# FrancescoScotti/Quadruped_gait_generation_ISMPC

Hardware: AMD Instinct MI355X
Metric: ISMPC QP solves/s (batch, N=100 horizon) (higher is better)
Workload: dtype f64; 1 GPU; Formulation B (MPCSolver::solve), trot plan Controller.cpp:89-97, N=100, S=35, F=10, fp64, global batch 65536 (65536 instances/GPU), nominal pre-roll + perturbation (SURVEY 8d); horizon=100, global_batch=65536, batch_per_gpu=65536

## Files before the change

quadruped_gait_generation_ismpc_amd/csrc/ismpc_b_common.hpp:

```cpp
#pragma once
#include <hip/hip_runtime.h>
#include <cmath>
#include "ismpc_tables.hpp"
#include "ismpc_wave_prims.hpp"

namespace {

using namespace ismpc_wave;

struct DevConst {
    int N, NP, NPs, S, F, nmid, npat, Fmax, rows, tick_divisor;
    double dt, cdt, mass, g, h_des, half_run, half_first, q_p, q_u, q_v, z_lo, z_hi, gate, eta;
    double inv_mass, dt_over_mass, inv_eta, sim_div, cdt_over_dt;
    const double *Hinv, *W, *midx, *midy, *midz, *tailx, *taily, *ftsp_t;
    const int *e_lo, *ne;
    const double *vtab, *tz, *tg, *dU, *SdU, *Wt, *SW;
    int flat;
    const double *HSt, *SHSt;
    const DevConst* sets; int nsets;
    const int* order;
    int* zflag;
    int* zseen;
    double* zpool; int* zbusy;
    int zslots, zcap, zldsq; size_t zstride;
    const double *vq;
    const double *tzg;
    const double *midxy;
    const double *vqT;
    const double *tzgT;
};

struct M2 { double a, b, c, d; };
__device__ __forceinline__ M2 mul(const M2& x, const M2& y)
{
    M2 r;
    r.a = fma(x.a, y.a, x.b * y.c); r.b = fma(x.a, y.b, x.b * y.d);
    r.c = fma(x.c, y.a, x.d * y.c); r.d = fma(x.c, y.b, x.d * y.d);
    return r;
}
template <int LANE>
__device__ __forceinline__ M2 readlane_m2(const M2& y)
{
    return (M2){readlane64<LANE>(y.a), readlane64<LANE>(y.b), readlane64<LANE>(y.c), readlane64<LANE>(y.d)};
}

__device__ __forceinline__ void sinhc_coshc(double w, double& P, double& Q)
{
    if (__builtin_expect(w <= 0.25, 1)) {
        P = 1.0 / 1307674368000.0;
        P = fma(P, w, 1.0 / 6227020800.0);
        P = fma(P, w, 1.0 / 39916800.0);
        P = fma(P, w, 1.0 / 362880.0);
        P = fma(P, w, 1.0 / 5040.0);
        P = fma(P, w, 1.0 / 120.0);
        P = fma(P, w, 1.0 / 6.0);
        P = fma(P, w, 1.0);
        Q = 1.0 / 20922789888000.0;
        Q = fma(Q, w, 1.0 / 87178291200.0);
        Q = fma(Q, w, 1.0 / 479001600.0);
        Q = fma(Q, w, 1.0 / 3628800.0);
        Q = fma(Q, w, 1.0 / 40320.0);
        Q = fma(Q, w, 1.0 / 720.0);
        Q = fma(Q, w, 1.0 / 24.0);
        Q = fma(Q, w, 0.5);
    } else {
        const double x = sqrt(w);
        P = sinh(x) / x;
        Q = (cosh(x) - 1.0) / w;
    }
}

__host__ __device__ inline size_t zscratch_bytes(int batch) { return 4 * (size_t)batch + 16; }
__device__ __forceinline__ int* zlist_of(unsigned char* zmark, int) { return reinterpret_cast<int*>(zmark); }
struct Walk { double sim; int mpc, ctl, fc; };
__device__ __forceinline__ Walk load_walk(const DevConst& c, const ismpc_tick_in* rec, int rollout_frame)
{
    Walk w; w.sim = rec->simulation_time; w.mpc = rec->mpc_iter; w.ctl = rec->control_iter; w.fc = rec->footstep_counter;
    if (rollout_frame >= 0) {
        if (w.fc >= 0 && w.fc < c.rows && w.sim >= c.ftsp_t[w.fc] - 1) { w.ctl = 0; w.mpc = 0; w.fc = w.fc + 1; }
        w.sim = (double)rollout_frame;
    }
    return w;
}
__device__ __forceinline__ int gate_tick(const DevConst& c, const Walk& w, int& idx)
{
    idx = 0;
    if ((w.ctl % c.tick_divisor) != 0) return ISMPC_ST_TICK_SKIPPED;
    const double t = (c.sim_div == 1.0) ? w.sim : w.sim / c.sim_div;
    if (!(t > -1.0) || !(t < 2.0e9)) return ISMPC_ST_BAD_INDEX;
    idx = (int)t;
    if (idx < 0 || idx + 2 * c.N > c.nmid || w.mpc < 0) return ISMPC_ST_BAD_INDEX;
// ... 49 lines not shown
```

quadruped_gait_generation_ismpc_amd/csrc/ismpc_b_group.hpp:

```cpp
#pragma once
#include "ismpc_b_affine.hpp"

namespace {

template <int CTRL, int BANK_MASK>
__device__ __forceinline__ double dpp64b(double old, double src)
{
    const int lo = __builtin_amdgcn_update_dpp(__double2loint(old), __double2loint(src), CTRL, 0xf, BANK_MASK, false);
    const int hi = __builtin_amdgcn_update_dpp(__double2hiint(old), __double2hiint(src), CTRL, 0xf, BANK_MASK, false);
    return __hiloint2double(hi, lo);
}
template <int CTRL, bool BOUND_ZERO>
__device__ __forceinline__ double dpp64n(double src)
{
    const int lo = __builtin_amdgcn_mov_dpp(__double2loint(src), CTRL, 0xf, 0xf, BOUND_ZERO);
    const int hi = __builtin_amdgcn_mov_dpp(__double2hiint(src), CTRL, 0xf, 0xf, BOUND_ZERO);
    return __hiloint2double(hi, lo);
}
template <int LPI> struct Grp;
template <> struct Grp<16> {
    static constexpr int STEPS = 4;
    __device__ static __forceinline__ double sum(double v)
    {
        v += dpp64n<0x121, false>(v); v += dpp64n<0x122, false>(v); v += dpp64n<0x124, false>(v); v += dpp64n<0x128, false>(v);
// ... 59 lines not shown
    }
    template <int K> __device__ static __forceinline__ double shl0(double v, int li)
    {
        if constexpr (K == 2) return dpp64b<0x104, 0x5>(0.0, v);
        else { const double t = dpp64n<0x100 + (1 << K), true>(v); return (li + (1 << K) < 8) ? t : 0.0; }
    }
    __device__ static __forceinline__ double bcast0(double v)
    {
        v = dpp64b<0x000, 0xf>(v, v); v = dpp64b<0x114, 0xa>(v, v);
        return v;
    }
    __device__ static __forceinline__ double next_or(double fill, double v, int li)
    {
        const double t = dppv<0x101, 0xf, false>(fill, v);
        return (li == 7) ? fill : t;
    }
};
template <int LPI, int K>
__device__ __forceinline__ void grp_scan_step(M2& y, int li)
{
    if constexpr (LPI == 32 && K == 4) {
        const bool g1 = (threadIdx.x & 32) != 0, low = li < 16;
        const double ya = g1 ? readlane64<48>(y.a) : readlane64<16>(y.a), yb = g1 ? readlane64<48>(y.b) : readlane64<16>(y.b);
        const double yc = g1 ? readlane64<48>(y.c) : readlane64<16>(y.c), yd = g1 ? readlane64<48>(y.d) : readlane64<16>(y.d);
        const double ta = low ? ya - 1.0 : 0.0, tb = low ? yb : 0.0, tc = low ? yc : 0.0, td = low ? yd - 1.0 : 0.0;
        M2 r;
        r.a = fma(ta, y.a, fma(tb, y.c, y.a)); r.b = fma(ta, y.b, fma(tb, y.d, y.b));
        r.c = fma(tc, y.a, fma(td, y.c, y.c)); r.d = fma(tc, y.b, fma(td, y.d, y.d));
        y = r;
    } else
    if constexpr (K < Grp<LPI>::STEPS) {
        const double ta = Grp<LPI>::template shl0<K>(y.a - 1.0, li), tb = Grp<LPI>::template shl0<K>(y.b, li);
        const double tc = Grp<LPI>::template shl0<K>(y.c, li), td = Grp<LPI>::template shl0<K>(y.d - 1.0, li);
        M2 r;
        r.a = fma(ta, y.a, fma(tb, y.c, y.a)); r.b = fma(ta, y.b, fma(tb, y.d, y.b));
        r.c = fma(tc, y.a, fma(td, y.c, y.c)); r.d = fma(tc, y.b, fma(td, y.d, y.d));
        y = r;
    }
}

template <int R> constexpr int midm() { return R | 1; }
template <int R, int LPI> constexpr int wave_lds_double2() { return (64 / LPI) * LPI * midm<R>(); }
template <int R, int LPI> constexpr int wave_lds_double2_fb() { return wave_lds_double2<R, LPI>() > (Z_LDS_DOUBLES + 1) / 2 ? wave_lds_double2<R, LPI>() : (Z_LDS_DOUBLES + 1) / 2; }

#ifndef ISMPC_KF_INLINE
#define ISMPC_KF_INLINE 0
#endif
#ifndef ISMPC_KF_MAIN
#define ISMPC_KF_MAIN 0
#endif
#ifndef ISMPC_KF_ROLLOUT
#define ISMPC_KF_ROLLOUT 0
#endif
template <int R, int LPI, int KF, bool SW = false>
__device__ __forceinline__ bool tick_group_core(const DevConst& c, const int lane, const QState& s, QOut& o, double* __restrict__ u_traj_inst,
                                                double2* __restrict__ lds_wave)
{
    constexpr int NT = ismpc::Tables::NT;
    const int N = c.N;
    const int li = lane & (LPI - 1);
    const double dt = c.dt;
    const Walk& w = s.w;
    const double x0 = s.x, y0 = s.y, z0 = s.z, xd0 = s.xd, yd0 = s.yd, zd0 = s.zd;
    const DevConst* P = SW ? c.sets + (s.ps >= 0 ? s.ps : 0) : nullptr;
    const double* p_vqT = SW ? P->vqT : c.vqT;
    const double p_z_lo = SW ? P->z_lo : c.z_lo, p_z_hi = SW ? P->z_hi : c.z_hi;
    const double p_inv_mass = SW ? P->inv_mass : c.inv_mass, p_inv_eta = SW ? P->inv_eta : c.inv_eta;
    const double p_half_run = SW ? P->half_run : c.half_run, p_half_first = SW ? P->half_first : c.half_first;
    const double* p_tailx = SW ? P->tailx : c.tailx; const double* p_taily = SW ? P->taily : c.taily;
    const double p_dt_over_mass = SW ? P->dt_over_mass : c.dt_over_mass, p_h_des = SW ? P->h_des : c.h_des;
    int idx;
    const int gate_status = gate_tick(c, w, idx) | ((SW && s.ps < 0) ? ISMPC_ST_BAD_INDEX : 0);
    int status = gate_status;
    const bool run = gate_status == 0;
    if (!run) idx = 0;
    const int n0 = li * R;
    STAMP_DECL;
    STAMP(1);

    const int pat = (run && w.fc > 1 && w.mpc < c.npat) ? w.mpc : c.npat;
    const double2* T = reinterpret_cast<const double2*>(p_vqT) + (size_t)pat * (R * 3 * LPI) + li;
    constexpr int MIDM = midm<R>();
    double2* Lm = lds_wave + (lane / LPI) * (LPI * MIDM);
#pragma unroll
    for (int k = 0; k < R; ++k) {
        const int j = k * LPI + li;
        Lm[(j / R) * MIDM + (j % R)] = reinterpret_cast<const double2*>(c.midxy)[min(idx + j, c.nmid - 1)];
    }
    double u[R], su[R];
    double smin = INFINITY, smax = -INFINITY;
#pragma unroll
    for (int r = 0; r < R; ++r) {
        const double2 t01 = T[(3 * r) * LPI], t23 = T[(3 * r + 1) * LPI], t45 = T[(3 * r + 2) * LPI];
        u[r] = fma(zd0, t23.x, fma(z0, t01.y, t01.x));
        su[r] = fma(zd0, t45.y, fma(z0, t45.x, t23.y));
        if (n0 + r < N) { smin = fmin(smin, su[r]); smax = fmax(smax, su[r]); }
    }
    if (!c.flat) {
        int elo = 0, ne = 0;
        if (pat < c.npat) { elo = c.e_lo[pat]; ne = c.ne[pat]; }
        const int pp = pat < c.npat ? pat : 0;
        int nemax = 0;
#pragma unroll
        for (int g = 0; g < 64; g += LPI) nemax = max(nemax, __builtin_amdgcn_readlane(ne, g));
        const double* dUr = (SW ? P->dU : c.dU) + (size_t)idx * NT;
        const double* sUr = (SW ? P->SdU : c.SdU) + (size_t)idx * NT;
        double du[R], ds[R];
#pragma unroll
        for (int r = 0; r < R; ++r) { du[r] = dUr[n0 + r]; ds[r] = sUr[n0 + r]; }
        for (int e = 0; e < nemax; ++e) {
            const bool on = e < ne;
            const double ue = on ? dUr[elo + e] : 0.0;
            const double* wr = (SW ? P->Wt : c.Wt) + ((size_t)pp * c.Fmax + (on ? e : 0)) * NT + n0;
            const double* sr = (SW ? P->SW : c.SW) + ((size_t)pp * c.Fmax + (on ? e : 0)) * NT + n0;
#pragma unroll
            for (int r = 0; r < R; ++r) { du[r] = fma(-wr[r], ue, du[r]); ds[r] = fma(-sr[r], ue, ds[r]); }
        }
        smin = INFINITY; smax = -INFINITY;
#pragma unroll
        for (int r = 0; r < R; ++r) {
            const int n = n0 + r;
            u[r] += du[r]; su[r] += ds[r];
            if (n >= elo && n < elo + ne) u[r] = 0.0;
            if (n < N) { smin = fmin(smin, su[r]); smax = fmax(smax, su[r]); }
        }
    }
    const double zlo_t = p_z_lo - 1e-11 * fmax(1.0, fabs(p_z_lo)), zhi_t = p_z_hi + 1e-11 * fmax(1.0, fabs(p_z_hi));
    const bool viol = smin < zlo_t || smax > zhi_t;
    const unsigned long long vmask = __builtin_amdgcn_ballot_w64(viol);
    const bool deferred = run && (((vmask >> (lane & (64 - LPI))) & ((1ull << LPI) - 1ull)) != 0ull);
    if (deferred) status |= ISMPC_ST_Z_INEQ_ACTIVE;

    double ch1[R], s1[R], s2[R], lam0_l = 0.0;
    bool big = false, mid = false;
    {
        double wv_[R], le_[R];
#pragma unroll
        for (int r = 0; r < R; ++r) {
            const double2 tq = reinterpret_cast<const double2*>(c.tzgT)[r * LPI + li];
            const double zpos = su[r] + fma(tq.x, zd0, z0) + tq.y;
            const double zacc = fma(p_inv_mass, u[r], -c.g);
            const double lam = (c.g + zacc) * frcp(zpos);
            if (r == 0) lam0_l = lam;
            le_[r] = (lam < c.gate) ? 0.0 : lam;
            const double dtn = (n0 + r < N) ? dt : 0.0;
            wv_[r] = le_[r] * dtn * dtn;
            s1[r] = dtn;
            big = big || (wv_[r] > 0.25);
            mid = mid || (wv_[r] > 0.004);
        }
        if (__builtin_amdgcn_ballot_w64(mid) == 0) {
#pragma unroll
            for (int r = 0; r < R; ++r) {
                const double wv = wv_[r];
                double P = 1.0 / 5040.0, Q = 1.0 / 40320.0;
                P = fma(P, wv, 1.0 / 120.0);         Q = fma(Q, wv, 1.0 / 720.0);
                P = fma(P, wv, 1.0 / 6.0);           Q = fma(Q, wv, 1.0 / 24.0);
                P = fma(P, wv, 1.0);                 Q = fma(Q, wv, 0.5);
                ch1[r] = wv * Q; s1[r] = s1[r] * P; s2[r] = le_[r] * s1[r];
            }
        } else {
            const bool gmid = ((__builtin_amdgcn_ballot_w64(mid) >> (lane & (64 - LPI))) & ((LPI == 64) ? ~0ull : ((1ull << LPI) - 1ull))) != 0ull;
#pragma unroll
            for (int r = 0; r < R; ++r) {
                const double wv = wv_[r], dtn = s1[r];
                double P = 1.0 / 1307674368000.0, Q = 1.0 / 20922789888000.0;
                P = fma(P, wv, 1.0 / 6227020800.0);  Q = fma(Q, wv, 1.0 / 87178291200.0);
                P = fma(P, wv, 1.0 / 39916800.0);    Q = fma(Q, wv, 1.0 / 479001600.0);
                P = fma(P, wv, 1.0 / 362880.0);      Q = fma(Q, wv, 1.0 / 3628800.0);
                P = gmid ? fma(P, wv, 1.0 / 5040.0) : 1.0 / 5040.0;   Q = gmid ? fma(Q, wv, 1.0 / 40320.0) : 1.0 / 40320.0;
                P = fma(P, wv, 1.0 / 120.0);         Q = fma(Q, wv, 1.0 / 720.0);
                P = fma(P, wv, 1.0 / 6.0);           Q = fma(Q, wv, 1.0 / 24.0);
                P = fma(P, wv, 1.0);                 Q = fma(Q, wv, 0.5);
                ch1[r] = wv * Q; s1[r] = dtn * P; s2[r] = le_[r] * s1[r];
                if (__builtin_amdgcn_ballot_w64(big) != 0 && wv > 0.25) {
                    const double x = sqrt(wv);
                    ch1[r] = cosh(x) - 1.0; s1[r] = dtn * (sinh(x) / x); s2[r] = le_[r] * s1[r];
                }
            }
        }
    }
    M2 Y = (M2){1.0 + ch1[0], s1[0], s2[0], 1.0 + ch1[0]};
#pragma unroll
    for (int r = 1; r < R; ++r) Y = mul((M2){1.0 + ch1[r], s1[r], s2[r], 1.0 + ch1[r]}, Y);
    STAMP(2);
    grp_scan_step<LPI, 0>(Y, li); grp_scan_step<LPI, 1>(Y, li); grp_scan_step<LPI, 2>(Y, li); grp_scan_step<LPI, 3>(Y, li);
    grp_scan_step<LPI, 4>(Y, li);
    const double ie = p_inv_eta;
    const double cva = fma(ie, Y.c, Y.a), cvb = fma(ie, Y.d, Y.b);
    double c0 = Grp<LPI>::next_or(1.0, cva, li), c1 = Grp<LPI>::next_or(ie, cvb, li);
    double a[R];
#pragma unroll
    for (int r = R - 1; r >= 0; --r) {
        a[r] = -fma(c0, ch1[r], c1 * s2[r]);
        const double k0 = fma(c0, ch1[r], fma(c1, s2[r], c0)), k1 = fma(c1, ch1[r], fma(c0, s1[r], c1));
        c0 = k0; c1 = k1;
    }
    const double h = (w.fc > 1) ? p_half_run : p_half_first;
    double q0 = 0.0, s_ax = 0.0, s_ay = 0.0, mx0 = 0.0, my0 = 0.0;
    __builtin_amdgcn_fence(__ATOMIC_SEQ_CST, "wavefront"); __builtin_amdgcn_wave_barrier();
#pragma unroll
    for (int r = 0; r < R; ++r) {
        const int n = n0 + r;
        const double2 mq = Lm[li * MIDM + r];
        const double mx = (n < N) ? mq.x : 0.0, my = (n < N) ? mq.y : 0.0;
        if (r == 0) { mx0 = mx; my0 = my; }
        q0 = fma(a[r], a[r], q0); s_ax = fma(a[r], mx, s_ax); s_ay = fma(a[r], my, s_ay);
    }
    q0 = Grp<LPI>::sum(q0); s_ax = Grp<LPI>::sum(s_ax); s_ay = Grp<LPI>::sum(s_ay);
    const double bpx = Grp<LPI>::bcast0((p_tailx[idx] - fma(cva, x0, cvb * xd0)) - s_ax);
    const double bpy = Grp<LPI>::bcast0((p_taily[idx] - fma(cva, y0, cvb * yd0)) - s_ay);
    const double sgx = (bpx < 0.0) ? -1.0 : 1.0, sgy = (bpy < 0.0) ? -1.0 : 1.0;
    STAMP(3);
    const double Tq[2] = { fabs(bpx), fabs(bpy) };
    const double iq0 = frcp(q0);
    double tau[2] = { Tq[0] * iq0, Tq[1] * iq0 };
    int its[2] = {1, 1}, prev[2] = {0, 0};
    bool live[2] = {true, true};
    int st3 = 0;
    if (!(q0 > 0.0)) {
#pragma unroll
        for (int ax = 0; ax < 2; ++ax) {
            tau[ax] = (Tq[ax] > 0.0) ? INFINITY : 0.0;
            if (Tq[ax] > 1e-300) st3 |= (ax == 0 ? ISMPC_ST_X_INFEASIBLE : ISMPC_ST_Y_INFEASIBLE);
        }
    }
    if constexpr (KF == 0) {
        for (int it = 0; it < N + 2; ++it) {
            if (__builtin_amdgcn_ballot_w64(live[0] || live[1]) == 0ull) break;
#pragma unroll
            for (int ax = 0; ax < 2; ++ax) {
                if (__builtin_amdgcn_ballot_w64(live[ax]) == 0ull) continue;
                int cl = 0;
#pragma unroll
                for (int r = 0; r < R; ++r) cl += (tau[ax] * fabs(a[r]) >= h) ? 1 : 0;
                const int cnt = Grp<LPI>::sum_i(cl);
                if (live[ax] && cnt == prev[ax]) live[ax] = false;
                if (__builtin_amdgcn_ballot_w64(live[ax]) == 0ull) continue;
                double ssat = 0.0, qfree = 0.0;
#pragma unroll
                for (int r = 0; r < R; ++r) {
                    const double ab = fabs(a[r]);
                    const bool sat = tau[ax] * ab >= h;
                    const double ms = sat ? 1.0 : 0.0, mf = sat ? 0.0 : 1.0;
                    ssat = fma(ms, ab, ssat); qfree = fma(mf, a[r] * a[r], qfree);
                }
                ssat = Grp<LPI>::sum(ssat); qfree = Grp<LPI>::sum(qfree);
                if (live[ax]) {
                    ++its[ax];
                    const double rem = fma(-h, ssat, Tq[ax]);
                    if (!(qfree > 0.0)) {
                        if (rem > fma(h * ssat, 1e-12, 1e-300)) st3 |= (ax == 0 ? ISMPC_ST_X_INFEASIBLE : ISMPC_ST_Y_INFEASIBLE);
                        tau[ax] = INFINITY; live[ax] = false;
                    } else {
                        const double tn = rem * frcp(qfree);
                        if (!(tn > tau[ax])) live[ax] = false;
                        else { tau[ax] = tn; prev[ax] = cnt; }
                    }
                }
            }
        }
    } else {
        for (int it = 0; it < N + 2; ++it) {
            if (__builtin_amdgcn_ballot_w64(live[0] || live[1]) == 0ull) break;
            int cl[2] = {0, 0};
            double ssat[2] = {0.0, 0.0}, qfree[2] = {0.0, 0.0};
#pragma unroll
            for (int ax = 0; ax < 2; ++ax) {
#pragma unroll
                for (int r = 0; r < R; ++r) {
                    const bool sat = tau[ax] * fabs(a[r]) >= h;
                    cl[ax] += sat ? 1 : 0; ssat[ax] += sat ? fabs(a[r]) : 0.0;
                    const double a2 = a[r] * a[r]; qfree[ax] += sat ? 0.0 : a2;
                }
            }
            const int cnt0 = Grp<LPI>::sum_i(cl[0]), cnt1 = Grp<LPI>::sum_i(cl[1]);
            ssat[0] = Grp<LPI>::sum(ssat[0]); ssat[1] = Grp<LPI>::sum(ssat[1]);
            qfree[0] = Grp<LPI>::sum(qfree[0]); qfree[1] = Grp<LPI>::sum(qfree[1]);
#pragma unroll
            for (int ax = 0; ax < 2; ++ax) {
                const int cnt = ax == 0 ? cnt0 : cnt1;
                if (live[ax] && cnt == prev[ax]) live[ax] = false;
                if (live[ax]) {
                    ++its[ax];
                    const double rem = fma(-h, ssat[ax], Tq[ax]);
                    if (!(qfree[ax] > 0.0)) {
                        if (rem > fma(h * ssat[ax], 1e-12, 1e-300)) st3 |= (ax == 0 ? ISMPC_ST_X_INFEASIBLE : ISMPC_ST_Y_INFEASIBLE);
                        tau[ax] = INFINITY; live[ax] = false;
                    } else {
                        const double tn = rem * frcp(qfree[ax]);
                        if (!(tn > tau[ax])) live[ax] = false;
                        else { tau[ax] = tn; prev[ax] = cnt; }
                    }
                }
            }
        }
    }

    STAMP(4);
    o.x = x0; o.y = y0; o.z = z0; o.xd = xd0; o.yd = yd0; o.zd = zd0;
    o.uz0 = 0.0; o.ux0 = 0.0; o.uy0 = 0.0; o.itx = 0; o.ity = 0;
    if (li == 0 && run) {
        o.uz0 = u[0];
        o.z = fma(dt, zd0, z0);
        o.zd = fma(p_dt_over_mass, o.uz0, zd0) - dt * c.g;
        if (isnan(o.z)) { o.z = p_h_des; status |= ISMPC_ST_Z_NAN; }
        if (isnan(o.zd)) { o.zd = 0.0; status |= ISMPC_ST_Z_NAN; }
        const double A0a = 1.0 + ch1[0], A0b = s1[0], A0c = s2[0];
        if (lam0_l > c.gate) {
            status |= st3; o.itx = its[0]; o.ity = its[1];
            const double sa0 = (a[0] < 0.0) ? -1.0 : 1.0;
            o.ux0 = fma(sgx * sa0, (fabs(a[0]) > 0.0) ? fmin(tau[0] * fabs(a[0]), h) : 0.0, mx0);
            o.uy0 = fma(sgy * sa0, (fabs(a[0]) > 0.0) ? fmin(tau[1] * fabs(a[0]), h) : 0.0, my0);
        } else status |= ISMPC_ST_FLIGHT;
        o.x  = fma(1.0 - A0a, o.ux0, fma(A0a, x0, A0b * xd0));
        o.xd = fma(-A0c, o.ux0, fma(A0c, x0, A0a * xd0));
        o.y  = fma(1.0 - A0a, o.uy0, fma(A0a, y0, A0b * yd0));
        o.yd = fma(-A0c, o.uy0, fma(A0c, y0, A0a * yd0));
    }
    o.status = status;
    if (u_traj_inst) {
        const bool stage3 = run && Grp<LPI>::bcast0(lam0_l) > c.gate;
#pragma unroll
        for (int r = 0; r < R; ++r) {
            const int n = n0 + r;
            if (n < N) {
                double vx = 0.0, vy = 0.0;
                if (stage3) {
                    const double sa = (a[r] < 0.0) ? -1.0 : 1.0;
                    vx = fma(sgx * sa, (fabs(a[r]) > 0.0) ? fmin(tau[0] * fabs(a[r]), h) : 0.0, c.midx[idx + n]);
                    vy = fma(sgy * sa, (fabs(a[r]) > 0.0) ? fmin(tau[1] * fabs(a[r]), h) : 0.0, c.midy[idx + n]);
                }
                u_traj_inst[n] = run ? u[r] : 0.0; u_traj_inst[N + n] = vx; u_traj_inst[2 * N + n] = vy;
            }
        }
    }
    return deferred;
}

template <int R, int LPI, int KF, bool SW = false>
__device__ __forceinline__ bool tick_group_body(const DevConst& c, const int gi_raw, const int batch, const int lane,
                                                const ismpc_tick_in* __restrict__ in_ro, ismpc_tick_in* state_rw,
                                                ismpc_tick_out* __restrict__ out, double* __restrict__ u_traj,
                                                int rollout_frame, unsigned char* zmark, int launch_id, double2* __restrict__ lds_wave, int* zlist = nullptr)
{
    const bool valid = gi_raw < batch;
    const int gi = valid ? gi_raw : batch - 1;
    STAMP_DECL;
    STAMP(0);
    const ismpc_tick_in* rec = ((rollout_frame >= 0) ? state_rw : in_ro) + gi;
    QState s;
    s.w = load_walk(c, rec, rollout_frame);
    s.x = rec->com_pos[0]; s.y = rec->com_pos[1]; s.z = rec->com_pos[2];
    s.xd = rec->com_vel[0]; s.yd = rec->com_vel[1]; s.zd = rec->com_vel[2];
    s.ps = 0;
    if (SW) { const int ps = rec->reserved; s.ps = (ps >= 0 && ps < c.nsets) ? ps : -1; }
    QOut o;
    const bool deferred = tick_group_core<R, LPI, KF, SW>(c, lane, s, o, (u_traj && valid) ? u_traj + (size_t)gi * 3 * c.N : nullptr, lds_wave);
    if ((lane & (LPI - 1)) == 0 && valid) {
        if (out) store_record(out + gi, o);
        if (deferred) {
            if (c.zseen) *c.zseen = launch_id;
            if (zlist) { const int slot = atomicAdd(c.zflag, 1); if (slot < batch) zlist[slot] = gi; }
        }
        if (rollout_frame >= 0 && !deferred) store_feedback(c, state_rw + gi, o, s.w);
    }
    STAMP(5);
    return deferred && valid;
}

#ifndef ISMPC_QUAD_WAVES
#define ISMPC_QUAD_WAVES 4
#endif
__device__ __forceinline__ int sweep_vblock(int b, int nb)
{
    const int q = nb >> 3, r = nb & 7, x = b & 7;
    return x * q + min(x, r) + (b >> 3);
}
template <bool SW> __device__ __forceinline__ int slot_instance(const DevConst& c, int slot, int batch)
{
    if (SW) { if (c.order) return slot < batch ? c.order[slot] : batch; }
    return slot;
}
template <int R, int LPI, bool SW = false>
__global__ __launch_bounds__(64 * ISMPC_QUAD_WAVES)
void ismpc_tick_quad(const DevConst c, const ismpc_tick_in* __restrict__ in_ro, ismpc_tick_in* state_rw,
                     ismpc_tick_out* __restrict__ out, double* __restrict__ u_traj, int batch, int rollout_frame,
                     unsigned char* zmark, int launch_id)
{
    constexpr int IPW = 64 / LPI;
    __shared__ double2 lds_mid[ISMPC_QUAD_WAVES][wave_lds_double2<R, LPI>()];
    const int lane = threadIdx.x & 63;
    const int wv = __builtin_amdgcn_readfirstlane(threadIdx.x >> 6);
    const int blk = (SW && c.order) ? sweep_vblock(blockIdx.x, gridDim.x) : (int)blockIdx.x;
    const int wave = blk * ISMPC_QUAD_WAVES + wv;
    if (wave * IPW >= batch) return;
    tick_group_body<R, LPI, ISMPC_KF_MAIN, SW>(c, slot_instance<SW>(c, wave * IPW + lane / LPI, batch), batch, lane, in_ro, state_rw, out, u_traj, rollout_frame, zmark, launch_id, lds_mid[wv],
                                               zmark ? zlist_of(zmark, batch) : nullptr);
}

template <int R, int LPI, int RW>
__global__ __launch_bounds__(64 * ISMPC_QUAD_WAVES, 2)
void ismpc_tick_quad_inline(const DevConst c, const ismpc_tick_in* __restrict__ in_ro, ismpc_tick_in* state_rw,
                            ismpc_tick_out* __restrict__ out, double* __restrict__ u_traj, int batch, int rollout_frame,
                            unsigned char* zmark, int launch_id, const DevConst* __restrict__ cdev)
{
    constexpr int IPW = 64 / LPI;
    __shared__ double2 lds_mid[ISMPC_QUAD_WAVES][wave_lds_double2_fb<R, LPI>()];
    const int lane = threadIdx.x & 63;
    const int wv = __builtin_amdgcn_readfirstlane(threadIdx.x >> 6);
    const int wave = blockIdx.x * ISMPC_QUAD_WAVES + wv;
    if (wave * IPW >= batch) return;
    const bool def = tick_group_body<R, LPI, ISMPC_KF_INLINE>(c, wave * IPW + lane / LPI, batch, lane, in_ro, state_rw, out, u_traj, rollout_frame, zmark, launch_id, lds_mid[wv]);
    unsigned long long m = __builtin_amdgcn_ballot_w64(def);
    if (m == 0ull) return;
    __builtin_amdgcn_fence(__ATOMIC_SEQ_CST, "wavefront");
// ... 143 lines not shown
```

quadruped_gait_generation_ismpc_amd/csrc/ismpc_hip.hip:

```cpp
#include <hip/hip_runtime.h>
#include <cmath>
#include <cstring>
#include <cstdlib>
#include <string>
#include <vector>
#include <new>
#include <algorithm>
#include <type_traits>
#include "ismpc_tables.hpp"
#include "ismpc_sweep.hpp"
#include "ismpc_host.hpp"

#pragma clang fp contract(off)

#include "ismpc_b_common.hpp"
#include "ismpc_b_dense.hpp"
#include "ismpc_b_affine.hpp"
#include "ismpc_b_group.hpp"

namespace {

thread_local std::string g_err = "";
int fail(int code, const std::string& msg) { g_err = msg; return code; }
#define HIP_TRY(expr) ISMPC_HIP_TRY(fail, expr)
// ... 242 lines not shown
            const ismpc_params& a = params[0]; const ismpc_params& b = params[k];
            if (a.N != b.N || a.S != b.S || a.F != b.F || a.M != b.M || a.mpc_dt != b.mpc_dt || a.control_dt != b.control_dt || a.g != b.g || a.lambda_gate != b.lambda_gate)
                return fail(ISMPC_E_INVALID, "the parameter sets of a sweep share N, S, F, M, mpc_dt, control_dt, g and lambda_gate");
            if (!(b.mass > 0) || !(b.h_des > 0) || !(b.q_u > 0) || b.q_p < 0 || b.q_v < 0) return fail(ISMPC_E_INVALID, "sweep: mass, h_des, q_u must be positive, q_p and q_v non-negative");
        }
    }
    int ndev = 0;
    if (hipGetDeviceCount(&ndev) != hipSuccess || ndev <= 0)
        return fail(ISMPC_E_NO_DEVICE, "no HIP device visible: the ISMPC hot path has no CPU fallback");
    if (device < 0 || device >= ndev) return fail(ISMPC_E_INVALID, "device ordinal out of range");
    ismpc_handle* h = new (std::nothrow) ismpc_handle();
    if (!h) return fail(ISMPC_E_ALLOC, "out of host memory");
    std::string err;
    int rc = ismpc::build_tables(*params, ftsp, rows, h->t, err);
    if (rc != ISMPC_OK) { delete h; return fail(rc, err); }
    h->device = device;
    if (const char* fw = std::getenv("ISMPC_WAVES")) {
        const int v = std::atoi(fw);
        if (v == 4 || v == 8 || v == 16) h->force_waves = v;
    }
    if (const char* pth = std::getenv("ISMPC_PATH")) { h->dense_path = std::strcmp(pth, "dense") == 0; h->quad_path = std::strcmp(pth, "wave") != 0 && !h->dense_path; }
    if (const char* zf = std::getenv("ISMPC_Z_FALLBACK")) h->z_fallback = std::atoi(zf) != 0;
    if (const char* lp = std::getenv("ISMPC_LPI")) { const int v = std::atoi(lp); if (v == 8 || v == 16 || v == 32) { h->lpi = v; h->lpi_auto = false; } }
    if (const char* ro = std::getenv("ISMPC_ROLLOUT")) h->kernel_rollout = std::strcmp(ro, "host") != 0;
    if (sweep) {
        h->sweep = true; h->lpi = 16; h->lpi_auto = false; h->quad_path = true; h->dense_path = false;
        h->sets.assign(params, params + K); h->ftsp.assign(ftsp, ftsp + (size_t)rows * 4);
    }
    DeviceGuard guard_(device);
    if (guard_.err != hipSuccess) { delete h; return fail(ISMPC_E_NO_DEVICE, std::string("hipSetDevice: ") + hipGetErrorString(guard_.err)); }
    { hipDeviceProp_t prop; h->cus = (hipGetDeviceProperties(&prop, device) == hipSuccess) ? prop.multiProcessorCount : 0; }
    if (const char* fu = std::getenv("ISMPC_ONE_LAUNCH")) h->one_launch = std::max(0, std::min(3, std::atoi(fu)));
    const ismpc::Tables& t = h->t;
    DevConst& c = h->c;
    c.N = t.p.N; c.NP = t.NP; c.NPs = t.NP + 2; c.S = t.p.S; c.F = t.p.F; c.nmid = t.nmid; c.npat = t.npat;
    c.Fmax = t.Fmax; c.rows = t.rows; c.tick_divisor = t.tick_divisor;
    c.dt = t.p.mpc_dt; c.cdt = t.p.control_dt; c.mass = t.p.mass; c.g = t.p.g; c.h_des = t.p.h_des;
    c.half_run = t.p.foot_width / 2; c.half_first = t.p.first_step_halfwidth;
    c.q_p = t.p.q_p; c.q_u = t.p.q_u; c.q_v = t.p.q_v; c.z_lo = t.p.z_ineq_lo; c.z_hi = t.p.z_ineq_hi;
    c.gate = t.p.lambda_gate; c.eta = t.eta;
    c.inv_mass = 1.0 / t.p.mass; c.dt_over_mass = t.p.mpc_dt / t.p.mass; c.inv_eta = 1.0 / t.eta;
    c.sim_div = t.p.mpc_dt / t.p.control_dt; c.cdt_over_dt = t.p.control_dt / t.p.mpc_dt;
    rc = upload(h, t.Hinv, &c.Hinv);
    if (rc == ISMPC_OK) rc = upload(h, t.W, &c.W);
    if (rc == ISMPC_OK) rc = upload(h, t.midx, &c.midx);
    if (rc == ISMPC_OK) rc = upload(h, t.midy, &c.midy);
    if (rc == ISMPC_OK) rc = upload(h, t.midz, &c.midz);
    if (rc == ISMPC_OK) rc = upload(h, t.tailx, &c.tailx);
    if (rc == ISMPC_OK) rc = upload(h, t.taily, &c.taily);
    if (rc == ISMPC_OK) rc = upload(h, t.ftsp_t, &c.ftsp_t);
    if (rc == ISMPC_OK) rc = upload(h, t.e_lo, &c.e_lo);
    if (rc == ISMPC_OK) rc = upload(h, t.ne, &c.ne);
    if (rc == ISMPC_OK) rc = upload(h, t.vtab, &c.vtab);
    if (rc == ISMPC_OK) rc = upload(h, t.tz, &c.tz);
    if (rc == ISMPC_OK) rc = upload(h, t.tg, &c.tg);
    if (rc == ISMPC_OK) rc = upload(h, t.dU, &c.dU);
    if (rc == ISMPC_OK) rc = upload(h, t.SdU, &c.SdU);
    if (rc == ISMPC_OK) rc = upload(h, t.Wt, &c.Wt);
    if (rc == ISMPC_OK) rc = upload(h, t.SW, &c.SW);
    if (rc == ISMPC_OK) rc = upload(h, t.HSt, &c.HSt);
    if (rc == ISMPC_OK) rc = upload(h, t.SHSt, &c.SHSt);
    if (rc == ISMPC_OK) { std::vector<int> zf(4, 0); const int* zp = nullptr; rc = upload(h, zf, &zp); c.zflag = const_cast<int*>(zp); }
    if (rc == ISMPC_OK) {
        void* hp = nullptr; void* dp = nullptr;
        if (hipHostMalloc(&hp, 64, hipHostMallocMapped) == hipSuccess && hipHostGetDevicePointer(&dp, hp, 0) == hipSuccess) {
            h->zseen_host = static_cast<int*>(hp); *h->zseen_host = 0; c.zseen = static_cast<int*>(dp);
        } else { if (hp) (void)hipHostFree(hp); (void)hipGetLastError(); c.zseen = nullptr; }
    }
    if (rc == ISMPC_OK) {
        c.zslots = 256; c.zcap = t.p.N; c.zldsq = Z_LDS_Q;
        if (const char* e = std::getenv("ISMPC_Z_LDS_Q")) c.zldsq = std::min(Z_LDS_Q, std::max(1, std::atoi(e)));
        c.zstride = (size_t)c.zcap * c.zcap + 4 * (size_t)c.zcap + ismpc::Tables::NT + ((size_t)c.zcap + 1) / 2 + 8;
        std::vector<int> busy(c.zslots, 0); const int* bp = nullptr;
        rc = upload(h, busy, &bp); c.zbusy = const_cast<int*>(bp);
        if (rc == ISMPC_OK) {
            void* zp = nullptr;
            if (hipMalloc(&zp, c.zstride * c.zslots * sizeof(double)) != hipSuccess) rc = fail(ISMPC_E_ALLOC, "fallback pool allocation failed");
            else { h->dev_allocs.push_back(zp); c.zpool = static_cast<double*>(zp); }
        }
    }
    if (rc == ISMPC_OK) {
        constexpr int NTq = ismpc::Tables::NT;
        const size_t npp = t.vtab.size() / (6 * (size_t)NTq);
        std::vector<double> vq(t.vtab.size()), tzg(2 * (size_t)NTq), mxy(2 * t.midx.size());
        for (size_t pp = 0; pp < npp; ++pp)
            for (int k = 0; k < 6; ++k)
                for (int n = 0; n < NTq; ++n) vq[(pp * NTq + n) * 6 + k] = t.vtab[(pp * 6 + k) * NTq + n];
        for (int n = 0; n < NTq; ++n) { tzg[2 * n] = t.tz[n]; tzg[2 * n + 1] = t.tg[n]; }
        for (size_t n = 0; n < t.midx.size(); ++n) { mxy[2 * n] = t.midx[n]; mxy[2 * n + 1] = t.midy[n]; }
        rc = upload(h, vq, &c.vq);
        if (rc == ISMPC_OK) rc = upload(h, tzg, &c.tzg);
        if (rc == ISMPC_OK) rc = upload(h, mxy, &c.midxy);
        if (rc == ISMPC_OK && t.p.N <= 128) {
            for (int pass = 0; pass < ((h->lpi_auto || sweep) ? 3 : 1) && rc == ISMPC_OK; ++pass) {
                const int lpi = pass == 0 ? h->lpi : (pass == 1 ? 32 : 8), R = quad_R(t.p.N, lpi);
                std::vector<double> vqT(npp * (size_t)R * 3 * lpi * 2), tzgT((size_t)R * lpi * 2);
                for (size_t pp = 0; pp < npp; ++pp)
                    for (int r = 0; r < R; ++r)
                        for (int k = 0; k < 3; ++k)
                            for (int li = 0; li < lpi; ++li) {
                                const int n = li * R + r;
                                const size_t dst = (((pp * R + r) * 3 + k) * lpi + li) * 2;
                                vqT[dst] = vq[(pp * NTq + n) * 6 + 2 * k]; vqT[dst + 1] = vq[(pp * NTq + n) * 6 + 2 * k + 1];
                            }
                for (int r = 0; r < R; ++r)
                    for (int li = 0; li < lpi; ++li) { const int n = li * R + r; tzgT[((size_t)r * lpi + li) * 2] = t.tz[n]; tzgT[((size_t)r * lpi + li) * 2 + 1] = t.tg[n]; }
                rc = upload(h, vqT, pass == 0 ? &c.vqT : (pass == 1 ? &h->vqT32 : &h->vqT8));
                if (rc == ISMPC_OK) rc = upload(h, tzgT, pass == 0 ? &c.tzgT : (pass == 1 ? &h->tzgT32 : &h->tzgT8));
            }
        }
    }
    c.flat = t.flat ? 1 : 0;
    if (rc != ISMPC_OK) { ismpc_destroy(h); return rc; }
    if (const char* hm = std::getenv("ISMPC_HOST_MODE")) h->host_mode = std::atoi(hm) & 3;
    if (hipStreamCreateWithFlags(&h->own_stream, hipStreamNonBlocking) != hipSuccess || hipEventCreate(&h->ev0) != hipSuccess ||
        hipEventCreate(&h->ev1) != hipSuccess) { ismpc_destroy(h); return fail(ISMPC_E_NO_DEVICE, "stream/event creation failed"); }
    if (sweep) {
        std::string serr;
        const char* lp8 = std::getenv("ISMPC_LPI");
        const bool lanes8 = !(lp8 && std::atoi(lp8) == 16);
        rc = ismpc::sweep_build(params, K, h->t, c.midx, c.midy, c.midz, c.e_lo, c.ne, 16, quad_R(t.p.N, 16), lanes8 ? 8 : 0, quad_R(t.p.N, 8), h->own_stream, h->sw, h->dev_allocs, serr);
        if (rc != ISMPC_OK) { ismpc_destroy(h); return fail(rc, serr); }
        std::vector<DevConst> cs((size_t)K, h->c);
        for (int k = 0; k < K; ++k) {
            DevConst& d = cs[k]; const ismpc_params& q = params[k];
            const double eta = std::sqrt(q.g / q.h_des);
            d.mass = q.mass; d.h_des = q.h_des; d.half_run = q.foot_width / 2; d.half_first = q.first_step_halfwidth;
            d.q_p = q.q_p; d.q_u = q.q_u; d.q_v = q.q_v; d.z_lo = q.z_ineq_lo; d.z_hi = q.z_ineq_hi; d.eta = eta;
            d.inv_mass = 1.0 / q.mass; d.dt_over_mass = q.mpc_dt / q.mass; d.inv_eta = 1.0 / eta;
            d.vtab = h->sw.vtab + (size_t)k * h->sw.s_vtab; d.vqT = h->sw.vqT + (size_t)k * h->sw.s_vqT;
            d.Wt = h->sw.Wt + (size_t)k * h->sw.s_W; d.SW = h->sw.SW + (size_t)k * h->sw.s_W;
            d.HSt = h->sw.HSt + (size_t)k * h->sw.s_HS; d.SHSt = h->sw.SHSt + (size_t)k * h->sw.s_HS;
            if (h->sw.dU) { d.dU = h->sw.dU + (size_t)k * h->sw.s_dU; d.SdU = h->sw.SdU + (size_t)k * h->sw.s_dU; }
            d.tailx = h->sw.tailx + (size_t)k * h->sw.s_tail; d.taily = h->sw.taily + (size_t)k * h->sw.s_tail;
            d.Hinv = nullptr; d.W = nullptr; d.vq = nullptr; d.sets = nullptr; d.nsets = 0;
        }
        void* sp = nullptr;
        if (hipMalloc(&sp, sizeof(DevConst) * (size_t)K) != hipSuccess) { ismpc_destroy(h); return fail(ISMPC_E_ALLOC, "sweep: set records allocation failed"); }
        h->dev_allocs.push_back(sp);
        if (hipMemcpy(sp, cs.data(), sizeof(DevConst) * (size_t)K, hipMemcpyHostToDevice) != hipSuccess) { ismpc_destroy(h); return fail(ISMPC_E_NO_DEVICE, "sweep: set records upload failed"); }
        h->c.sets = static_cast<const DevConst*>(sp); h->c.nsets = K;
        if (h->sw.vqT2) {
            for (int k = 0; k < K; ++k) cs[k].vqT = h->sw.vqT2 + (size_t)k * h->sw.s_vqT2;
            void* sp8 = nullptr;
            if (hipMalloc(&sp8, sizeof(DevConst) * (size_t)K) != hipSuccess) { ismpc_destroy(h); return fail(ISMPC_E_ALLOC, "sweep: set records allocation failed"); }
            h->dev_allocs.push_back(sp8);
            if (hipMemcpy(sp8, cs.data(), sizeof(DevConst) * (size_t)K, hipMemcpyHostToDevice) != hipSuccess) { ismpc_destroy(h); return fail(ISMPC_E_NO_DEVICE, "sweep: set records upload failed"); }
            h->sets8 = static_cast<const DevConst*>(sp8);
        }
    }
    {
        void* cp = nullptr;
        if (hipMalloc(&cp, sizeof(DevConst)) != hipSuccess) { ismpc_destroy(h); return fail(ISMPC_E_ALLOC, "constants allocation failed"); }
        h->dev_allocs.push_back(cp); h->c_dev = static_cast<DevConst*>(cp);
        if (hipMemcpy(cp, &h->c, sizeof(DevConst), hipMemcpyHostToDevice) != hipSuccess) { ismpc_destroy(h); return fail(ISMPC_E_NO_DEVICE, "constants upload failed"); }
    }
    *out = h;
    return ISMPC_OK;
}

int ismpc_create(const ismpc_params* params, const double* ftsp, int rows, int device, ismpc_handle** out)
{
    return create_impl(params, 1, false, ftsp, rows, device, out);
}

int ismpc_create_sweep(const ismpc_params* params, int n_sets, const double* ftsp, int rows, int device, ismpc_handle** out)
{
    return create_impl(params, n_sets, true, ftsp, rows, device, out);
}

int ismpc_sweep_bind(ismpc_handle* h, int batch, const ismpc_tick_in* in_dev, void* stream)
{
// ... 311 lines not shown
```

quadruped_gait_generation_ismpc_amd/csrc/ismpc_tables.cpp:

```cpp
#include "ismpc_tables.hpp"
#include <cmath>
#include <algorithm>

namespace ismpc {

typedef long double ld;

static bool cholesky(std::vector<ld>& a, int n)
{
    for (int j = 0; j < n; ++j) {
        ld s = a[(size_t)j*n+j];
        for (int k = 0; k < j; ++k) s -= a[(size_t)j*n+k]*a[(size_t)j*n+k];
        if (!(s > 0)) return false;
        ld ljj = sqrtl(s);
        a[(size_t)j*n+j] = ljj;
        for (int i = j + 1; i < n; ++i) {
            ld t = a[(size_t)i*n+j];
            for (int k = 0; k < j; ++k) t -= a[(size_t)i*n+k]*a[(size_t)j*n+k];
            a[(size_t)i*n+j] = t / ljj;
        }
    }
    return true;
}

static void chol_inverse(const std::vector<ld>& L, int n, std::vector<ld>& inv)
{
    std::vector<ld> Li((size_t)n*n, 0);
    for (int j = 0; j < n; ++j) {
        Li[(size_t)j*n+j] = 1 / L[(size_t)j*n+j];
        for (int i = j + 1; i < n; ++i) {
            ld s = 0;
            for (int k = j; k < i; ++k) s -= L[(size_t)i*n+k]*Li[(size_t)k*n+j];
            Li[(size_t)i*n+j] = s / L[(size_t)i*n+i];
        }
    }
    inv.assign((size_t)n*n, 0);
    for (int i = 0; i < n; ++i)
        for (int j = 0; j <= i; ++j) {
            ld s = 0;
            for (int k = i; k < n; ++k) s += Li[(size_t)k*n+i]*Li[(size_t)k*n+j];
            inv[(size_t)i*n+j] = s; inv[(size_t)j*n+i] = s;
        }
}

int build_tables(const ismpc_params& p, const double* ftsp, int rows, Tables& t, std::string& err)
{
    if (!ftsp || rows < 2) { err = "footstep plan needs at least 2 rows"; return ISMPC_E_INVALID; }
    if (p.N < 1 || p.N > 256) { err = "horizon N must be in [1, 256]"; return p.N > 256 ? ISMPC_E_UNSUPPORTED : ISMPC_E_INVALID; }
    if (p.S < 0 || p.F < 1 || p.S + p.F > 4096) { err = "S must be >= 0 and F >= 1"; return ISMPC_E_INVALID; }
    if (!(p.mpc_dt > 0) || !(p.control_dt > 0) || !(p.mass > 0) || !(p.g > 0) || !(p.h_des > 0)) {
        err = "mpc_dt, control_dt, mass, g, h_des must be positive"; return ISMPC_E_INVALID;
    }
    if (!(p.q_u > 0) || p.q_p < 0 || p.q_v < 0) { err = "weights: q_u > 0, q_p >= 0, q_v >= 0"; return ISMPC_E_INVALID; }
    if ((int)(100 * p.mpc_dt) <= 0) { err = "(int)(100*mpc_dt) is 0: the reference's tick gate (MPCSolver.cpp:214) divides by it"; return ISMPC_E_INVALID; }

    t.p = p;
    t.eta = std::sqrt(p.g / p.h_des);
    t.rows = rows;
    const int N = p.N, S = p.S, F = p.F;
    t.nmid = rows * (S + F);
    t.NP = (N + 15) / 16 * 16;
    t.npat = S + F;
    t.Fmax = F;
    t.tick_divisor = (int)(100 * p.mpc_dt);
    const ld dt = p.mpc_dt, m = p.mass;

    std::vector<ld> H((size_t)N*N);
    const ld cs = dt*dt/m, cv = dt/m;
    for (int i = 0; i < N; ++i)
        for (int j = 0; j <= i; ++j) {
            ld a = 0;
            for (int k = i + 1; k < N; ++k) a += (ld)(k - i) * (ld)(k - j);
            ld b = (ld)(N - 1 - i);
            ld v = (ld)p.q_p * cs*cs * a + (ld)p.q_v * cv*cv * b + (i == j ? (ld)p.q_u : 0);
            H[(size_t)i*N+j] = v; H[(size_t)j*N+i] = v;
        }
    std::vector<ld> L = H;
    if (!cholesky(L, N)) { err = "vertical Hessian is not positive definite"; return ISMPC_E_NUMERIC; }
    std::vector<ld> Hinv;
    chol_inverse(L, N, Hinv);
    t.Hinv.assign((size_t)t.NP*t.NP, 0.0);
    for (int i = 0; i < N; ++i)
        for (int j = 0; j < N; ++j) t.Hinv[(size_t)i*t.NP+j] = (double)Hinv[(size_t)i*N+j];

    t.e_lo.assign(t.npat, 0); t.ne.assign(t.npat, 0);
    t.W.assign((size_t)t.npat * t.Fmax * t.NP, 0.0);
    std::vector<ld> Wld((size_t)t.npat * t.Fmax * N, 0);
    for (int it = 0; it < t.npat; ++it) {
        int lo, hi;
        if (it < S) { lo = S - it; hi = std::min(S + F, N) - it; } else { lo = 0; hi = std::min(S + F - it, N); }
        if (hi <= lo) { lo = 0; hi = 0; }
        int cnt = hi - lo;
        t.e_lo[it] = lo; t.ne[it] = cnt;
        if (cnt == 0) continue;
        std::vector<ld> G((size_t)cnt*cnt), Gi;
        for (int a = 0; a < cnt; ++a)
            for (int b = 0; b < cnt; ++b) G[(size_t)a*cnt+b] = Hinv[(size_t)(lo+a)*N + (lo+b)];
        if (!cholesky(G, cnt)) { err = "equality Schur complement is not positive definite"; return ISMPC_E_NUMERIC; }
        chol_inverse(G, cnt, Gi);
        for (int e = 0; e < cnt; ++e)
            for (int n = 0; n < N; ++n) {
                ld s = 0;
                for (int a = 0; a < cnt; ++a) s += Hinv[(size_t)n*N + (lo+a)] * Gi[(size_t)a*cnt+e];
                t.W[((size_t)it*t.Fmax + e)*t.NP + n] = (double)s;
                Wld[((size_t)it*t.Fmax + e)*N + n] = s;
            }
    }

    t.midx.assign(t.nmid, 0.0); t.midy.assign(t.nmid, 0.0); t.midz.assign(t.nmid, 0.0);
    std::vector<double>* col[3] = { &t.midx, &t.midy, &t.midz };
    for (int i = 0; i < rows - 1; ++i)
        for (int c = 0; c < 3; ++c) {
            const double a = ftsp[i*4+c], b = ftsp[(i+1)*4+c];
            for (int r = 0; r < S; ++r) (*col[c])[i*(S+F)+r] = a * 1.0;
            for (int r = 0; r < F; ++r) (*col[c])[i*(S+F)+S+r] = a * 1.0 + (b - a) * ((double)r / (double)F);
        }
    t.ftsp_t.resize(rows);
    for (int i = 0; i < rows; ++i) t.ftsp_t[i] = ftsp[i*4+3];

    std::vector<double> deltas(N);
    for (int i = 0; i < N; ++i) deltas[i] = std::exp(-p.mpc_dt * t.eta * i);
    t.tailx.assign(t.nmid, 0.0); t.taily.assign(t.nmid, 0.0);
    for (int idx = 0; idx + 2*N <= t.nmid; ++idx) {
        double sx = 0, sy = 0;
        for (int i = 0; i < N; ++i) {
            const double wgt = t.eta * p.mpc_dt * deltas[i];
            sx += wgt * t.midx[idx+N+i]; sy += wgt * t.midy[idx+N+i];
        }
        t.tailx[idx] = sx; t.taily[idx] = sy;
    }

    const int NT = Tables::NT;
    auto apply_St = [&](const std::vector<ld>& r, std::vector<ld>& o, bool vel) {
        o.assign(N, 0);
        if (vel) { ld acc = 0; for (int i = N - 1; i >= 0; --i) { o[i] = cv * acc; acc += r[i]; } }
        else { ld t1 = 0, t2 = 0; for (int i = N - 1; i >= 0; --i) { o[i] = cs * t2; t1 += r[i]; t2 += t1; } }
// ... 87 lines not shown
```

Baseline: 1.509 billion ticks/s (1 tick = one MPCSolver::solve = 3 QPs: vertical + x + y).

## Pad midpoint table, drop clamps, add two-lane KF=2 breakpoint loop, hoist u store

```diff
diff --git a/quadruped_gait_generation_ismpc_amd/csrc/ismpc_b_common.hpp b/quadruped_gait_generation_ismpc_amd/csrc/ismpc_b_common.hpp
--- a/quadruped_gait_generation_ismpc_amd/csrc/ismpc_b_common.hpp
+++ b/quadruped_gait_generation_ismpc_amd/csrc/ismpc_b_common.hpp
@@ -7,6 +7,8 @@
 namespace {
 
 using namespace ismpc_wave;
+
+constexpr int MID_PAD = 128;
 
 struct DevConst {
     int N, NP, NPs, S, F, nmid, npat, Fmax, rows, tick_divisor;
diff --git a/quadruped_gait_generation_ismpc_amd/csrc/ismpc_b_group.hpp b/quadruped_gait_generation_ismpc_amd/csrc/ismpc_b_group.hpp
--- a/quadruped_gait_generation_ismpc_amd/csrc/ismpc_b_group.hpp
+++ b/quadruped_gait_generation_ismpc_amd/csrc/ismpc_b_group.hpp
@@ -165,10 +165,12 @@
     const double2* T = reinterpret_cast<const double2*>(p_vqT) + (size_t)pat * (R * 3 * LPI) + li;
     constexpr int MIDM = midm<R>();
     double2* Lm = lds_wave + (lane / LPI) * (LPI * MIDM);
+    static_assert(LPI * R <= MID_PAD, "the midpoint table's padding must cover the staged window");
+    const double2* Mw = reinterpret_cast<const double2*>(reinterpret_cast<const char*>(c.midxy) + (size_t)((unsigned)(idx + li) * 16u));
 #pragma unroll
     for (int k = 0; k < R; ++k) {
         const int j = k * LPI + li;
-        Lm[(j / R) * MIDM + (j % R)] = reinterpret_cast<const double2*>(c.midxy)[min(idx + j, c.nmid - 1)];
+        Lm[(j / R) * MIDM + (j % R)] = Mw[k * LPI];
     }
     double u[R], su[R];
     double smin = INFINITY, smax = -INFINITY;
@@ -213,6 +215,12 @@
     const unsigned long long vmask = __builtin_amdgcn_ballot_w64(viol);
     const bool deferred = run && (((vmask >> (lane & (64 - LPI))) & ((1ull << LPI) - 1ull)) != 0ull);
     if (deferred) status |= ISMPC_ST_Z_INEQ_ACTIVE;
+    if (u_traj_inst) {
+#pragma unroll
+        for (int r = 0; r < R; ++r)
+            if (n0 + r < N) u_traj_inst[n0 + r] = run ? u[r] : 0.0;
+    }
+    const double uz0 = u[0];
 
     double ch1[R], s1[R], s2[R], lam0_l = 0.0;
     bool big = false, mid = false;
@@ -284,11 +292,9 @@
     __builtin_amdgcn_fence(__ATOMIC_SEQ_CST, "wavefront"); __builtin_amdgcn_wave_barrier();
 #pragma unroll
     for (int r = 0; r < R; ++r) {
-        const int n = n0 + r;
         const double2 mq = Lm[li * MIDM + r];
-        const double mx = (n < N) ? mq.x : 0.0, my = (n < N) ? mq.y : 0.0;
-        if (r == 0) { mx0 = mx; my0 = my; }
-        q0 = fma(a[r], a[r], q0); s_ax = fma(a[r], mx, s_ax); s_ay = fma(a[r], my, s_ay);
+        if (r == 0) { mx0 = mq.x; my0 = mq.y; }
+        q0 = fma(a[r], a[r], q0); s_ax = fma(a[r], mq.x, s_ax); s_ay = fma(a[r], mq.y, s_ay);
     }
     q0 = Grp<LPI>::sum(q0); s_ax = Grp<LPI>::sum(s_ax); s_ay = Grp<LPI>::sum(s_ay);
     const double bpx = Grp<LPI>::bcast0((p_tailx[idx] - fma(cva, x0, cvb * xd0)) - s_ax);
@@ -342,6 +348,46 @@
                     }
                 }
             }
+        }
+    } else if constexpr (KF == 2) {
+        for (int it = 0; it < 2 * (N + 2); ++it) {
+            const bool any = live[0] || live[1];
+            if (__builtin_amdgcn_ballot_w64(any) == 0ull) break;
+            const bool ony = !live[0];
+            const double tc = ony ? tau[1] : tau[0], Tc = ony ? Tq[1] : Tq[0];
+            const int pc = ony ? prev[1] : prev[0];
+            int cl = 0;
+#pragma unroll
+            for (int r = 0; r < R; ++r) cl += (tc * fabs(a[r]) >= h) ? 1 : 0;
+            const int cnt = Grp<LPI>::sum_i(cl);
+            bool lv = any && cnt != pc;
+            double tn = tc;
+            int bit = 0;
+            if (__builtin_amdgcn_ballot_w64(lv) != 0ull) {
+                double ssat = 0.0, qfree = 0.0;
+#pragma unroll
+                for (int r = 0; r < R; ++r) {
+                    const double ab = fabs(a[r]);
+                    const bool sat = tc * ab >= h;
+                    const double ms = sat ? 1.0 : 0.0, mf = sat ? 0.0 : 1.0;
+                    ssat = fma(ms, ab, ssat); qfree = fma(mf, a[r] * a[r], qfree);
+                }
+                ssat = Grp<LPI>::sum(ssat); qfree = Grp<LPI>::sum(qfree);
+                if (lv) {
+                    const double rem = fma(-h, ssat, Tc);
+                    if (!(qfree > 0.0)) {
+                        if (rem > fma(h * ssat, 1e-12, 1e-300)) bit = 1;
+                        tn = INFINITY; lv = false;
+                    } else {
+                        const double t1 = rem * frcp(qfree);
+                        if (!(t1 > tc)) lv = false;
+                        else tn = t1;
+                    }
+                    if (ony) ++its[1]; else ++its[0];
+                }
+            }
+            if (ony) { tau[1] = tn; live[1] = lv; if (lv) prev[1] = cnt; if (bit) st3 |= ISMPC_ST_Y_INFEASIBLE; }
+            else     { tau[0] = tn; live[0] = lv; if (lv) prev[0] = cnt; if (bit) st3 |= ISMPC_ST_X_INFEASIBLE; }
         }
     } else {
         for (int it = 0; it < N + 2; ++it) {
@@ -384,7 +430,7 @@
     o.x = x0; o.y = y0; o.z = z0; o.xd = xd0; o.yd = yd0; o.zd = zd0;
     o.uz0 = 0.0; o.ux0 = 0.0; o.uy0 = 0.0; o.itx = 0; o.ity = 0;
     if (li == 0 && run) {
-        o.uz0 = u[0];
+        o.uz0 = uz0;
         o.z = fma(dt, zd0, z0);
         o.zd = fma(p_dt_over_mass, o.uz0, zd0) - dt * c.g;
         if (isnan(o.z)) { o.z = p_h_des; status |= ISMPC_ST_Z_NAN; }
@@ -414,7 +460,7 @@
                     vx = fma(sgx * sa, (fabs(a[r]) > 0.0) ? fmin(tau[0] * fabs(a[r]), h) : 0.0, c.midx[idx + n]);
                     vy = fma(sgy * sa, (fabs(a[r]) > 0.0) ? fmin(tau[1] * fabs(a[r]), h) : 0.0, c.midy[idx + n]);
                 }
-                u_traj_inst[n] = run ? u[r] : 0.0; u_traj_inst[N + n] = vx; u_traj_inst[2 * N + n] = vy;
+                u_traj_inst[N + n] = vx; u_traj_inst[2 * N + n] = vy;
             }
         }
     }
diff --git a/quadruped_gait_generation_ismpc_amd/csrc/ismpc_hip.hip b/quadruped_gait_generation_ismpc_amd/csrc/ismpc_hip.hip
--- a/quadruped_gait_generation_ismpc_amd/csrc/ismpc_hip.hip
+++ b/quadruped_gait_generation_ismpc_amd/csrc/ismpc_hip.hip
@@ -348,12 +348,13 @@
     if (rc == ISMPC_OK) {
         constexpr int NTq = ismpc::Tables::NT;
         const size_t npp = t.vtab.size() / (6 * (size_t)NTq);
-        std::vector<double> vq(t.vtab.size()), tzg(2 * (size_t)NTq), mxy(2 * t.midx.size());
+        std::vector<double> vq(t.vtab.size()), tzg(2 * (size_t)NTq), mxy(2 * (t.midx.size() + MID_PAD), 0.0);
         for (size_t pp = 0; pp < npp; ++pp)
             for (int k = 0; k < 6; ++k)
                 for (int n = 0; n < NTq; ++n) vq[(pp * NTq + n) * 6 + k] = t.vtab[(pp * 6 + k) * NTq + n];
         for (int n = 0; n < NTq; ++n) { tzg[2 * n] = t.tz[n]; tzg[2 * n + 1] = t.tg[n]; }
         for (size_t n = 0; n < t.midx.size(); ++n) { mxy[2 * n] = t.midx[n]; mxy[2 * n + 1] = t.midy[n]; }
+        for (size_t n = t.midx.size(); n < t.midx.size() + MID_PAD && !t.midx.empty(); ++n) { mxy[2 * n] = t.midx.back(); mxy[2 * n + 1] = t.midy.back(); }
         rc = upload(h, vq, &c.vq);
         if (rc == ISMPC_OK) rc = upload(h, tzg, &c.tzg);
         if (rc == ISMPC_OK) rc = upload(h, mxy, &c.midxy);
diff --git a/quadruped_gait_generation_ismpc_amd/csrc/ismpc_tables.cpp b/quadruped_gait_generation_ismpc_amd/csrc/ismpc_tables.cpp
--- a/quadruped_gait_generation_ismpc_amd/csrc/ismpc_tables.cpp
+++ b/quadruped_gait_generation_ismpc_amd/csrc/ismpc_tables.cpp
@@ -52,6 +52,8 @@
         err = "mpc_dt, control_dt, mass, g, h_des must be positive"; return ISMPC_E_INVALID;
     }
     if (!(p.q_u > 0) || p.q_p < 0 || p.q_v < 0) { err = "weights: q_u > 0, q_p >= 0, q_v >= 0"; return ISMPC_E_INVALID; }
+    for (int i = 0; i < rows * 4; ++i)
+        if (!std::isfinite(ftsp[i])) { err = "footstep plan holds a non-finite entry"; return ISMPC_E_INVALID; }
     if ((int)(100 * p.mpc_dt) <= 0) { err = "(int)(100*mpc_dt) is 0: the reference's tick gate (MPCSolver.cpp:214) divides by it"; return ISMPC_E_INVALID; }
 
     t.p = p;
```

New measurement: 1.527 billion ticks/s (1 tick = one MPCSolver::solve = 3 QPs: vertical + x + y), median of 6. 1.2% higher.
